# EthanD11/RS-VIO

Hardware: AMD Instinct MI355X
Metric: stereo frames/sec (tracker+BA) on 752×480 EuRoC stream; BA ms/iter at window=10 (higher is better)
Workload: dtype f32 (tracker) / f64 (BA)

## Files before the change

### rs-vio_amd/csrc/ba.hip

```cpp
#include <rccl/rccl.h>

#include <algorithm>
#include <chrono>
#include <cmath>
#include <cstdlib>
#include <cstring>
#include <string>
#include <sys/resource.h>
#include <numeric>
#include <stdexcept>
#include <vector>

#include "common.hpp"

#include "ba_envelope.hpp"
#include "obs_pass.hpp"
#include "se3.hpp"
#include "wave.hpp"

#pragma clang fp contract(fast)

namespace rsvio {

namespace {

RSVIO_DBG_DECL
RSVIO_RT_DECL

constexpr int kMaxFree = 20;
static_assert(kMaxFree == rsvio_env::kMaxFree, "ba_envelope.hpp sizes env[] for the same camera system");
constexpr int kMaxN = 6 * kMaxFree;
enum { RV = 0, RGP = 6, RWR = 9, RUR = 18, RGR = 24, kRawF = 28 };
enum { LV = 0, LG = 6, kLmF = 12 };
// ... 114 lines not shown
    const int* dmap;
};

struct Work {
    double* pose[2];
    double* pw[2];
    const double* pose_init;
    const double* pw_init;
    double* raws[2];
    double* rawl[2];
    int* singular;
    const int* p2p_err;
    double* partA;
    double* partD;
    double* cpart;
    double* sys;
    double* dc;
    double* trial4;
    const LmState* st_prev;
    LmState* st;
    unsigned long long* tick;
};

__device__ __forceinline__ size_t sys_len(const Geometry& G) { return (size_t)G.n_pb * 36 + 12 * G.n_free + 2; }

constexpr int kP2PMax = 8;
constexpr int kP2PMsg = 8192;

struct P2P {
    double* peer[kP2PMax];
    int nranks, rank;
    int* xnw;
    int ll;
};

constexpr int kP2PWaves = 16384;
constexpr size_t kP2PTval = (size_t)2 * kP2PMax * kP2PMsg + 2 * kP2PMax;
constexpr size_t kP2PTflag = kP2PTval + (size_t)2 * kP2PMax * kP2PWaves * 4;
constexpr int kP2PLLMax = 16;
constexpr size_t kP2PLL = kP2PTflag + (size_t)2 * kP2PMax * kP2PWaves;
constexpr size_t kP2PLLSys = kP2PLL + (size_t)2 * kP2PMax * 2 * kP2PLLMax;
constexpr size_t kP2PBytes = sizeof(double) * (kP2PLLSys + (size_t)2 * kP2PMax * 2 * kP2PMsg);

__device__ __forceinline__ unsigned long long* p2p_flags(double* xbuf) {
    return reinterpret_cast<unsigned long long*>(xbuf + (size_t)2 * kP2PMax * kP2PMsg);
}
// ... 183 lines not shown
#pragma unroll
            for (int c = a; c < 3; ++c) L.V[k++] += wt * (J[0][a] * J[0][c] + J[1][a] * J[1][c]);
            L.gp[a] += J[0][a] * wr0 + J[1][a] * wr1;
        }
        if (fr) {
            int u = 0;
#pragma unroll
            for (int a = 0; a < 3; ++a) {
#pragma unroll
                for (int c = 0; c < 3; ++c) L.Wr[a * 3 + c] += wt * (J[0][6 + a] * J[0][c] + J[1][6 + a] * J[1][c]);
#pragma unroll
                for (int c = a; c < 3; ++c) L.Ur[u++] += wt * (J[0][6 + a] * J[0][6 + c] + J[1][6 + a] * J[1][6 + c]);
                L.gr[a] += J[0][6 + a] * wr0 + J[1][6 + a] * wr1;
            }
        }
    }
}

__device__ __forceinline__ void wave_sync() {
    __builtin_amdgcn_fence(__ATOMIC_SEQ_CST, "wavefront");
    __builtin_amdgcn_wave_barrier();
}

template <bool WAVE = false>
__device__ void store_linearization(const Work& Wk, int buf, int s, int lane, bool act, bool fr, int first, int nk,
                                    int l, const SlotLin& L, double (*sh)[64]) {
    if (act && fr) {
        double rec[kRawF];
#pragma unroll
        for (int i = 0; i < 6; ++i) rec[RV + i] = L.V[i];
#pragma unroll
        for (int i = 0; i < 3; ++i) rec[RGP + i] = L.gp[i];
#pragma unroll
        for (int i = 0; i < 9; ++i) rec[RWR + i] = L.Wr[i];
#pragma unroll
        for (int i = 0; i < 6; ++i) rec[RUR + i] = L.Ur[i];
#pragma unroll
        for (int i = 0; i < 3; ++i) rec[RGR + i] = L.gr[i];
        rec[27] = 0.0;
        double2* dst = reinterpret_cast<double2*>(Wk.raws[buf] + (size_t)s * kRawF);
#pragma unroll
        for (int i = 0; i < kRawF / 2; ++i) dst[i] = make_double2(rec[2 * i], rec[2 * i + 1]);
    }
#pragma unroll
    for (int i = 0; i < 6; ++i) sh[i][lane] = L.V[i];
#pragma unroll
    for (int i = 0; i < 3; ++i) sh[6 + i][lane] = L.gp[i];
    if constexpr (WAVE) wave_sync(); else __syncthreads();
// ... 178 lines not shown
        scan(R, true, base);
    }
    for (int i = total + tid; i < G.pair_stride; i += 256) out[i] = make_int4(-1, 0, 0, 0);
}

__global__ __launch_bounds__(256) void ba_stage_in(const uint4* src, uint4* __restrict__ dst, int n_words) {
    const int t = (int)(blockIdx.x * 256 + threadIdx.x), st = (int)(gridDim.x * 256);
    const int i0 = t, i1 = t + st;
    uint4 a, b;
    host_load2x16(src + min(i0, n_words - 1), src + min(i1, n_words - 1), a, b);
    if (i0 < n_words) dst[i0] = a;
    if (i1 < n_words) dst[i1] = b;
}

__global__ __launch_bounds__(256) void ba_build_layout(Geometry G, Prob Pr, SlotSrc S, int nb_slots, int4* hdr,
                                                       double2* huv, int4* pairs) {
    const int b = blockIdx.x;
    if (b < nb_slots)
        build_slots_body(G, Pr, S, hdr, huv, b);
    else
        build_pairs_body(G, Pr, S, pairs, b - nb_slots);
}

__device__ void linearize_body(const Geometry& G, const Prob& Pr, const Work& Wk, int w, int with_reset,
                               double lambda0) {
    __shared__ double sh[10][64];
    const int lane = threadIdx.x;
    const int s = 64 * w + lane;
    if (with_reset) {
        const int nt = G.n_wave * 64;
        for (int i = s; i < 7 * G.n_kf; i += nt) {
            Wk.pose[0][i] = Wk.pose_init[i];
            Wk.pose[1][i] = Wk.pose_init[i];
        }
        for (int i = s; i < 3 * G.n_lm; i += nt) {
            Wk.pw[0][i] = Wk.pw_init[i];
            Wk.pw[1][i] = Wk.pw_init[i];
        }
        if (s == 0) {
            Wk.tick[1] = wall_clock64();
            *Wk.singular = 0;
            LmState st{};
            st.lambda = lambda0;
            st.nu = 2.0;
            *Wk.st = st;
        }
    }
// ... 10 lines not shown
        const Pose P = pose_from7(pose0 + 7 * kf);
        const double* pwp = pw0 + 3 * l;
        const double p[3] = {pwp[0], pwp[1], pwp[2]};
        slot_linearize(G, P, p, h1.y, h1.z, uvq, fr, L);
    } else {
        const Pose P{};
        const double p[3] = {0.0, 0.0, 1.0};
        slot_linearize(G, P, p, 0, 0, uvq, false, L);
    }
    STAMP(12);
    store_linearization(Wk, 0, s, lane, act, fr, first, nk, l, L, sh);
    const double c = wave_sum_det(L.cost);
    if (lane == 0) {
        Wk.partA[w * kPartA] = c;
        Wk.partA[w * kPartA + 1] = 0.0;
    }
    STAMP(14);
}

__global__ __launch_bounds__(64) void ba_linearize(Geometry G, Prob Pr, Work Wk, double lambda0) {
    linearize_body(G, Pr, Wk, blockIdx.x, 1, lambda0);
}

__device__ void trial_scalars_wave(const Geometry& G, const Prob& Pr, const Work& Wk, const LmState& s,
                                   int include_poses, double out[4]) {
    const int lane = threadIdx.x & 63;
    constexpr int kU = 8;
    double4 pv[kU];
    const int wl = max(G.n_wave - 1, 0), el = 7 * G.n_kf - 1;
#pragma unroll
    for (int k = 0; k < kU; ++k)
        pv[k] = *reinterpret_cast<const double4*>(Wk.partD + (size_t)min(lane + 64 * k, wl) * kPartD);
    double p0[3], p1[3];
    int fi[3];
#pragma unroll
    for (int k = 0; k < 3; ++k) {
        const int e = min(lane + 64 * k, el);
        fi[k] = Pr.free_idx[e / 7];
        p0[k] = Wk.pose[0][e];
        p1[k] = Wk.pose[1][e];
    }
#pragma unroll
    for (int k = 0; k < kU; ++k)
        if (lane + 64 * k >= G.n_wave) pv[k] = make_double4(0.0, 0.0, 0.0, 0.0);
    bool fr[3];
#pragma unroll
    for (int k = 0; k < 3; ++k) fr[k] = include_poses && lane + 64 * k <= el && fi[k] >= 0;
// ... 121 lines not shown
                s.nu = 2.0;
                s.cost = s.new_cost;
            } else {
                s.lambda *= s.nu;
                s.nu *= 2.0;
                if (s.lambda > 1e32) {
                    s.status = RSVIO_LM_TRUST_REGION;
                    s.done = 1;
                }
            }
        }
    }
    if (!s.done && s.iter >= max_iter) {
        s.status = RSVIO_LM_MAX_ITERATIONS;
        s.done = 1;
    }
}

struct LmArgs {
    int max_iter;
    double cost_tol, param_tol;
};

__device__ LmState lm_decide(const Geometry& G, const Prob& Pr, const Work& Wk, const LmState* src, int pre_reduced,
                             const LmArgs& la, const P2P* PP = nullptr, const unsigned long long* xgen = nullptr,
                             int* err = nullptr) {
    LmState s = *src;
    double tv[4];
    if (pre_reduced == 4) {
        const int lane = threadIdx.x & 63, r = lane >> 2, i = lane & 3, nr = PP->nranks;
        const unsigned long long gen = *xgen;
        const unsigned g32 = (unsigned)gen;
        const unsigned long long* wv = p2p_ll(PP->peer[PP->rank], (int)(gen & 1), min(r, nr - 1)) + 2 * i;
        unsigned long long a = __hip_atomic_load(wv, __ATOMIC_RELAXED, __HIP_MEMORY_SCOPE_SYSTEM);
        unsigned long long b = __hip_atomic_load(wv + 1, __ATOMIC_RELAXED, __HIP_MEMORY_SCOPE_SYSTEM);
        for (int k = 0; k < 4; ++k) tv[k] = 0.0;
        if (s.pending && !s.done && s.solve_ok) {
            long long spins = 0;
            bool late = false;
            while (r < nr && !((unsigned)(a >> 32) == g32 && (unsigned)(b >> 32) == g32)) {
                if (++spins > (1ll << 25)) {
                    late = true;
                    break;
                }
                __builtin_amdgcn_s_sleep(1);
                a = __hip_atomic_load(wv, __ATOMIC_RELAXED, __HIP_MEMORY_SCOPE_SYSTEM);
                b = __hip_atomic_load(wv + 1, __ATOMIC_RELAXED, __HIP_MEMORY_SCOPE_SYSTEM);
            }
            if (late) atomicExch(err, 1);
            const double got = late ? 0.0 : __longlong_as_double((long long)((a & 0xffffffffull) | (b << 32)));
            for (int k = 0; k < 4; ++k) {
                double v = 0.0;
                for (int q = 0; q < nr; ++q) v += rl64(got, 4 * q + k);
                tv[k] = v;
            }
        }
    } else if (pre_reduced == 2) {
        const unsigned long long gen = *xgen;
        for (int k = 0; k < 4; ++k) tv[k] = 0.0;
        if (s.pending && !s.done && s.solve_ok) trial_scalars_p2p(G, Pr, Wk, s, *PP, gen, err, tv);
    } else if (pre_reduced) {
        for (int k = 0; k < 4; ++k) tv[k] = Wk.trial4[k];
    } else {
        trial_scalars_wave(G, Pr, Wk, s, 1, tv);
    }
    const double cost0 = Wk.sys[(size_t)G.n_pb * 36 + 12 * G.n_free];
    __asm__ volatile("" ::"v"(tv[0]), "v"(tv[1]), "v"(tv[2]), "v"(tv[3]), "v"(cost0));
    STAMP(29);
    if (s.pending && !s.done) {
        const double cost = s.iter == 0 ? cost0 : s.cost;
        lm_update(s, cost, tv, la.max_iter, la.cost_tol, la.param_tol);
        s.pending = 0;
    }
    return s;
}

__device__ __forceinline__ void slot_w(const double* rec, double W[18]) {
    const double* v = rec + RV;
    const double Vs[9] = {v[0], v[1], v[2], v[1], v[3], v[4], v[2], v[4], v[5]};
#pragma unroll
    for (int i = 0; i < 9; ++i) W[i] = Vs[i];
#pragma unroll
    for (int i = 0; i < 9; ++i) W[9 + i] = rec[RWR + i];
}

template <bool DIAG>
__device__ __forceinline__ void schur_pair(const Work& Wk, int cur, double lambda, int chol, int sa, int sb, int l,
                                           double (&acc)[kBlockF]) {
    const double2* ra = reinterpret_cast<const double2*>(Wk.raws[cur] + (size_t)sa * kRawF);
    const double2* rb = reinterpret_cast<const double2*>(Wk.raws[cur] + (size_t)sb * kRawF);
    const double2* rl = reinterpret_cast<const double2*>(Wk.rawl[cur] + (size_t)l * kLmF);
    constexpr int NA = DIAG ? kRawF / 2 : 9;
    double Ra[2 * NA], Rb[18], Lm[10];
#pragma unroll
    for (int i = 0; i < NA; ++i) {
        const double2 x = ra[i];
        Ra[2 * i] = x.x; Ra[2 * i + 1] = x.y;
    }
    if constexpr (!DIAG)
#pragma unroll
        for (int i = 0; i < 9; ++i) {
            const double2 y = rb[i];
            Rb[2 * i] = y.x; Rb[2 * i + 1] = y.y;
        }
#pragma unroll
    for (int i = 0; i < 5; ++i) {
        const double2 x = rl[i];
        Lm[2 * i] = x.x; Lm[2 * i + 1] = x.y;
    }
    double Wa[18], Wb[18];
// ... 25 lines not shown
            for (int c = 0; c < 3; ++c) {
                U[a * 6 + c] = Wa[a * 3 + c];
                U[(3 + a) * 6 + c] = Wa[(3 + a) * 3 + c];
                U[c * 6 + 3 + a] = Wa[(3 + a) * 3 + c];
            }
        const double* ur = Ra + RUR;
        const double Ur[9] = {ur[0], ur[1], ur[2], ur[1], ur[3], ur[4], ur[2], ur[4], ur[5]};
#pragma unroll
        for (int a = 0; a < 3; ++a)
#pragma unroll
            for (int c = 0; c < 3; ++c) U[(3 + a) * 6 + 3 + c] = Ur[a * 3 + c];
#pragma unroll
        for (int i = 0; i < 36; ++i) acc[i] += U[i];
#pragma unroll
        for (int a = 0; a < 6; ++a) {
            const double gca = a < 3 ? Ra[RGP + a] : Ra[RGR + a - 3];
            const double yg = fma(Ya[a * 3 + 2], Lm[LG + 2], fma(Ya[a * 3 + 1], Lm[LG + 1], Ya[a * 3] * Lm[LG]));
            acc[36 + a] += yg - gca;
            acc[42 + a] += gca;
        }
    }
}

template <bool DIAG>
__device__ __forceinline__ void schur_chunk_pairs(const Geometry& G, const Work& Wk, const LmState& s, const int4* pr,
                                                  int4 p1, int tid, double (&acc)[kBlockF]) {
    if (p1.x >= 0) schur_pair<DIAG>(Wk, s.cur, s.lambda, G.chol, p1.x, p1.y, p1.z, acc);
    for (int p = tid + kSchurThreads; p < G.pair_stride; p += kSchurThreads) {
        const int4 q = pr[p];
        if (q.x >= 0) schur_pair<DIAG>(Wk, s.cur, s.lambda, G.chol, q.x, q.y, q.z, acc);
    }
}

__device__ void schur_chunks_body(const Geometry& G, const Prob& Pr, const Work& Wk, const LmArgs& la,
                                  int pre_reduced, int c, const P2P* PP = nullptr,
                                  const unsigned long long* xgen = nullptr, int* err = nullptr) {
    __shared__ double red[kSchurThreads / 64][kBlockF];
    const int tid = threadIdx.x, lane = tid & 63, wave = tid >> 6;
    const int pb = c / kGrp, x = c % kGrp;
    RTSTAMP(0);
    STAMP(26);
    if (G.env_on) {
        int a = 0, r = pb;
        while (a < G.n_free && r >= G.n_free - a) {
            r -= G.n_free - a;
            ++a;
        }
        if (a < G.n_free && a + r > (int)G.env[a]) {
            if (tid < 36) Wk.cpart[(size_t)x * sys_len(G) + pb * 36 + tid] = 0.0;
            return;
        }
    }
    const int4* pr = Pr.pairs + (size_t)c * G.pair_stride;
    const int4 p1 = tid < G.pair_stride ? pr[tid] : make_int4(-1, 0, 0, 0);
    const int fa = Pr.pb_fa[pb];
    const bool diag = fa == Pr.pb_fb[pb];
    __shared__ LmState sd;
// ... 269 lines not shown
            const double piv = rl64(a[0], 0);
            bad = !(piv > 0.0) || !isfinite(piv);
            inv = rcp_f64(piv);
        }
        int seen = 0;
        double uq[CW];
#pragma unroll
        for (int jj = 0; jj < CW; ++jj) uq[jj] = 0.0;
        chol_pipe_step<NP, CW, WV, 0>(a, lane, Lc, Uc, progress, seen, bad, inv, uq, 0.0);
    }
    if (lane == 0) badw[WV] = bad ? 1 : 0;
#ifdef RSVIO_STAMPS
    if (lane == 0) g_dbg[24 + WV] = (unsigned long long)clock64();
#endif
}

__device__ __forceinline__ void k5_result(LmState* st, int ok, double d2, double gd) {
    st->solve_ok = ok;
    st->dc2 = d2;
    st->gcdc = gd;
    st->pending = 1;
}

template <int NF>
__device__ void k5_finish(const Geometry& G, const Work& Wk, double* A, double x, double gcl_v, int n, int lane,
                          const double (&p7)[7], int fidx) {
    LmState* st = Wk.st;
    const double d2 = wave_sum_det(x * x);
    const double gd = wave_sum_det(lane < n ? gcl_v * x : 0.0);
    __builtin_amdgcn_wave_barrier();
    if (lane < n) {
        Wk.dc[lane] = x;
        A[lane] = x;
    }
    __builtin_amdgcn_s_waitcnt(0xc07f);
    __builtin_amdgcn_wave_barrier();
    STAMP(4);
    if (lane < G.n_kf) {
        double* q = Wk.pose[1 - st->cur] + 7 * lane;
        if (fidx < 0) {
#pragma unroll
            for (int i = 0; i < 7; ++i) q[i] = p7[i];
        } else {
            double qv[7];
            se3_plus(p7, A + 6 * fidx, qv);
#pragma unroll
            for (int i = 0; i < 7; ++i) q[i] = qv[i];
        }
// ... 173 lines not shown
    static constexpr int NT = NP / 16 + 1;
    static constexpr int NPP = 16 * NT;
    static constexpr int NH = (NP + kMfPanel - 1) / kMfPanel;
};

constexpr int kMfMapLambda = 1 << 30;
inline void mf_dense_map(int nf, int n_pb, const int* pb_fa, const int* pb_fb, int* map, int np_target = 0,
                         int ld = kMfLd) {
    const int np = np_target > 0 ? np_target : 6 * nf;
    for (int pb = 0; pb < n_pb; ++pb)
        for (int k = 0; k < 36; ++k) {
            const int ra = k / 6, ca = k % 6, fa = pb_fa[pb], fb = pb_fb[pb];
            int v;
            if (fa == fb)
                v = ra >= ca ? ((6 * fa + ca) * ld + 6 * fa + ra) | (ra == ca ? kMfMapLambda : 0) : -1;
            else
                v = (6 * fa + ra) * ld + 6 * fb + ca;
            map[36 * pb + k] = v;
        }
    for (int i = 0; i < 6 * nf; ++i) map[36 * n_pb + i] = i * ld + np;
    for (int i = 0; i < 6 * nf; ++i) map[36 * n_pb + 6 * nf + i] = -2 - i;
}

template <int NF>
__device__ bool combine_mapped(const Geometry& G, const Prob& Pr, const Work& Wk, double* M, double* gsh,
                               const LmState* st, int* fail) {
    constexpr int NE = (NF * (NF + 1) / 2) * 36 + 12 * NF;
    constexpr int T = kK5Threads, kE = (NE + T - 1) / T;
    const size_t L = sys_len(G);
    const int ne = G.n_pb * 36 + 12 * G.n_free;
    const int tid = threadIdx.x;
    double v[kE][kGrp];
    int dst[kE];
#pragma unroll
    for (int i = 0; i < kE; ++i) {
        const int e = tid + T * i, ec = min(e, ne - 1);
        const int d = Pr.dmap[ec];
        dst[i] = e < ne ? d : -1;
#pragma unroll
        for (int x = 0; x < kGrp; ++x) v[i][x] = Wk.cpart[(size_t)x * L + ec];
    }
    double pa[16];
    int sing = 0;
    if (tid < 64) {
        const int wl = max(G.n_wave - 1, 0);
#pragma unroll
        for (int k = 0; k < 16; ++k) pa[k] = Wk.partA[min(tid + 64 * k, wl) * kPartA];
        sing = *Wk.singular;
    }
    const int done = st->done;
    const double lambda = st->lambda;
#pragma unroll
    for (int i = 0; i < kE; ++i)
#pragma unroll
        for (int x = 0; x < kGrp; ++x) __asm__ volatile("" ::"v"(v[i][x]));
    if (done) return true;
#pragma unroll
    for (int i = 0; i < kE; ++i) {
        double a = v[i][0];
#pragma unroll
        for (int x = 1; x < kGrp; ++x) a += v[i][x];
        const int d = dst[i];
        if (d >= 0) {
            if (d & kMfMapLambda) a += lambda;
            M[d & (kMfMapLambda - 1)] = a;
        } else if (d <= -2) {
            gsh[-2 - d] = a;
        }
    }
    if (tid < 64) {
        double c = 0.0;
#pragma unroll
        for (int k = 0; k < 16; ++k) c += tid + 64 * k < G.n_wave ? pa[k] : 0.0;
        for (int w = tid + 64 * 16; w < G.n_wave; w += 64) c += Wk.partA[w * kPartA];
        c = wave_sum_det(c);
        if (tid == 0) {
            Wk.sys[G.n_pb * 36 + 12 * G.n_free] = c;
            *fail = sing;
        }
    }
    return false;
}

template <int NF>
__device__ bool combine_p2p_ll(const Geometry& G, const Work& Wk, double* M, double* gsh, int* fail, const P2P& P,
                               unsigned long long* xgen, int* err,
                               const double (&v)[((NF * (NF + 1) / 2) * 36 + 12 * NF + kK5Threads - 1) / kK5Threads][kGrp],
                               const int (&dst)[((NF * (NF + 1) / 2) * 36 + 12 * NF + kK5Threads - 1) / kK5Threads],
                               const double (&pa)[16], int sing, double lambda, unsigned long long gen) {
    constexpr int NE = (NF * (NF + 1) / 2) * 36 + 12 * NF;
    constexpr int T = kK5Threads, kE = (NE + T - 1) / T;
    const int ne = G.n_pb * 36 + 12 * G.n_free;
// ... 514 lines not shown
    } else {
        bk_update<NF, K, NW - 1>(M, U + (K & 1) * 6 * LD, lane, wave - 1, env[K]);
    }
    if constexpr (K + 1 < NF) bk_steps<NF, K + 1, NW, KD>(M, U, Dsc, Lsc, a, tid, bad, env, Dv);
}

template <int NF, int NW, bool KD = false>
__device__ __forceinline__ void bk_factor(double* M, double* U, double* S, int tid, bool& bad,
                                          const unsigned char* env, double* Dv = nullptr) {
    using D = BkDims<NF>;
    double a[D::RPL][6];
    if ((tid >> 6) == 0) {
        const int lane = tid & 63;
#pragma unroll
        for (int h = 0; h < D::RPL; ++h) {
            const int r = lane + 64 * h < D::NPP ? lane + 64 * h : D::NPP - 1;
#pragma unroll
            for (int j = 0; j < 6; ++j) a[h][j] = M[j * D::LD + r];
        }
    }
    bk_steps<NF, 0, NW, KD>(M, U, S, S + 36, a, tid, bad, env, Dv);
}

template <int NF, bool LL = false>
__device__ void camera_solve_mfma_body(const Geometry& G, const Prob& Pr, const Work& Wk, int combine,
                                       const P2P* P = nullptr, unsigned long long* xgen = nullptr, int* err = nullptr) {
    static_assert(NF >= 1 && NF <= 10, "one row per lane: n <= 60");
    constexpr int NP = MfDims<NF>::NP, NPP = MfDims<NF>::NPP;
    __shared__ __attribute__((aligned(16))) double M[NPP * kMfLd];
    __shared__ __attribute__((aligned(16))) double Lf[NPP * kMfLd];
    __shared__ __attribute__((aligned(16))) double Up[2 * kMfPanel * kMfLd];
    __shared__ double gsh[NP];
    __shared__ int fail;
    RTSTAMP(4);
    LmState* st = Wk.st;
    const int tid = threadIdx.x, lane = tid & 63, wave = tid >> 6;
    const int nF = G.n_free, n = 6 * nF;
    const int SC0 = G.n_pb * 36 + 12 * nF;
    double p7b[2][7];
    int fidx = -1;
    if (wave == 0 && lane < G.n_kf) {
        fidx = Pr.free_idx[lane];
#pragma unroll
        for (int b = 0; b < 2; ++b)
#pragma unroll
            for (int i = 0; i < 7; ++i) p7b[b][i] = Wk.pose[b][7 * lane + i];
    } else {
#pragma unroll
        for (int b = 0; b < 2; ++b)
#pragma unroll
            for (int i = 0; i < 7; ++i) p7b[b][i] = i == 3 ? 1.0 : 0.0;
    }
    STAMP(0);
    if (combine == 2) {
        if (combine_p2p<NF, LL>(G, Pr, Wk, M, gsh, st, &fail, *P, xgen, err)) return;
    } else if (combine) {
        if (combine_mapped<NF>(G, Pr, Wk, M, gsh, st, &fail)) return;
    } else {
        if (st->done) return;
        const double* sys = Wk.sys;
        const int ne = G.n_pb * 36 + 12 * nF;
        for (int e = tid; e < ne; e += kK5Threads) {
            const int d = Pr.dmap[e];
            if (d >= 0)
                M[d & (kMfMapLambda - 1)] = sys[e];
            else if (d <= -2)
                gsh[-2 - d] = sys[e];
        }
        if (tid == 0) fail = sys[SC0 + 1] != 0.0;
    }
    const int cur = st->cur;
    double p7[7];
#pragma unroll
    for (int i = 0; i < 7; ++i) p7[i] = cur ? p7b[1][i] : p7b[0][i];
    if (n < NP) {
        for (int e = tid; e < NP * (NP + 1); e += kK5Threads) {
            const int c = e / (NP + 1), r = e - c * (NP + 1);
            if (r >= c && ((r >= n && r < NP) || (c >= n && c < NP))) M[c * kMfLd + r] = r == c ? 1.0 : 0.0;
// ... 33 lines not shown
        const double m = Lres[lj * kMfLd + j];
        lt[j] = lane < j ? m : 0.0;
    }
#pragma unroll
    for (int j = NP - 1; j >= 0; --j) yv = fma(-lt[j], rl64(yv, j), yv);
    STAMP(3);
    k5_finish<NF>(G, Wk, Up, lane < n ? yv : 0.0, gcl_v, n, lane, p7, fidx);
    RTSTAMP(5);
}

template <int NF>
__global__ __launch_bounds__(kK5Threads) void ba_camera_solve_mfma(Geometry G, Prob Pr, Work Wk, int combine) {
    camera_solve_mfma_body<NF>(G, Pr, Wk, combine);
}

template <int NF, bool LL>
__global__ __launch_bounds__(kK5Threads) void ba_camera_solve_mfma_p2p(Geometry G, Prob Pr, Work Wk, P2P P,
                                                                        unsigned long long* xgen, int* err) {
    camera_solve_mfma_body<NF, LL>(G, Pr, Wk, 2, &P, xgen, err);
}

constexpr int kBkWaves = 8;

template <int NF>
__device__ __forceinline__ void camera_solve_blk_body(const Geometry& G, const Prob& Pr, const Work& Wk, int combine) {
    using D = BkDims<NF>;
    constexpr int NP = D::NP, LD = D::LD;
    static_assert(NF > 10 && D::RPL == 2 && D::NPP <= LD, "the 11..20 free-keyframe solver");
    constexpr int T = 64 * kBkWaves;
    __shared__ __attribute__((aligned(16))) double M[16 * D::NTC * LD];
    __shared__ __attribute__((aligned(16))) double U[2 * 6 * LD];
    __shared__ __attribute__((aligned(16))) double S[72];
    __shared__ double gsh[NP];
    __shared__ double dcs[128];
    __shared__ int fail;
    LmState* st = Wk.st;
    const int tid = threadIdx.x, lane = tid & 63, wave = tid >> 6;
    const int nF = G.n_free, n = 6 * nF;
    const int ne = G.n_pb * 36 + 12 * nF;
    STAMP(0);
    double p7b[2][7];
    int fidx = -1;
#pragma unroll
    for (int b = 0; b < 2; ++b)
#pragma unroll
        for (int i = 0; i < 7; ++i) p7b[b][i] = i == 3 ? 1.0 : 0.0;
    if (wave == 0 && lane < G.n_kf) {
        fidx = Pr.free_idx[lane];
// ... 443 lines not shown
#pragma unroll
            for (int i = 0; i < 7; ++i) qd[i] = p7[i];
        } else {
            double qv[7];
            se3_plus(p7, dcs + 6 * fidx, qv);
#pragma unroll
            for (int i = 0; i < 7; ++i) qd[i] = qv[i];
        }
    }
    if (lane == 0) k5_result(st, 1, d2, gd);
    STAMP(5);
}

#ifndef RSVIO_EXPORT_FENCE
#define RSVIO_EXPORT_FENCE 0
#endif
__device__ __forceinline__ void export_done() {
#if RSVIO_EXPORT_FENCE
    __builtin_amdgcn_fence(__ATOMIC_RELEASE, "");
#else
    __builtin_amdgcn_s_waitcnt(kWaitStores);
#endif
}
template <bool FUSED, bool LAST = false>
__device__ void k6_body(const Geometry& G, const Prob& Pr, const Work& Wk, int w, int lane, double (*sh)[64],
                        double (*shp)[64], double (*shs)[64], const P2P* PP = nullptr,
                        unsigned long long gen = 0, unsigned long long* k6tag = nullptr,
                        unsigned long long* k6part = nullptr, double* hout = nullptr) {
    const int s = 64 * w + lane;
    const int4 h0 = Pr.slot_hdr[2 * s], h1 = Pr.slot_hdr[2 * s + 1];
    const double2 uvq[2] = {Pr.slot_uv[2 * s], Pr.slot_uv[2 * s + 1]};
    const LmState* st = Wk.st;
    const bool act = h1.y > 0;
    const int kf = h0.x, l = h0.y, first = act ? h0.z : lane, nk = act ? h0.w : 1;
    const bool fr = h1.x >= 0;
    const int kfc = act ? kf : 0, lc = act ? l : 0, fc = (act && fr) ? h1.x : 0;
    double recb[2][18], Lmb[2][10], pcb[2][3], p7b[2][7], d6[6];
#pragma unroll
    for (int b = 0; b < 2; ++b) {
        const double2* wr = reinterpret_cast<const double2*>(Wk.raws[b] + (size_t)s * kRawF);
#pragma unroll
        for (int i = 0; i < 9; ++i) {
            const double2 x = wr[i];
            recb[b][2 * i] = x.x; recb[b][2 * i + 1] = x.y;
        }
        const double2* lr = reinterpret_cast<const double2*>(Wk.rawl[b] + (size_t)lc * kLmF);
#pragma unroll
        for (int i = 0; i < 5; ++i) {
// ... 408 lines not shown
        if (threadIdx.x == 0) __hip_atomic_store(k6cnt, 0u, __ATOMIC_RELAXED, __HIP_MEMORY_SCOPE_AGENT);
        k6_last_push(G, Pr, Wk, P, xgen, gen, k6part, s);
    } else {
        const LmState s = *Wk.st;
        if (s.done || !s.solve_ok) return;
        k6_last_push(G, Pr, Wk, P, xgen, gen, k6part, s);
    }
}

__global__ __launch_bounds__(64) void ba_reduce_trial(Geometry G, Prob Pr, Work Wk, int include_poses) {
    const LmState s = *Wk.st;
    if (s.done) return;
    double v[4];
    trial_scalars_wave(G, Pr, Wk, s, include_poses, v);
    if (threadIdx.x == 0)
        for (int k = 0; k < 4; ++k) Wk.trial4[k] = v[k];
}

constexpr int kK7Threads = 256;
#ifndef RSVIO_K7_BLOCKS
#define RSVIO_K7_BLOCKS 16
#endif
constexpr int kK7Blocks = RSVIO_K7_BLOCKS;
__device__ __forceinline__ void lm_decide_body(const Geometry& G, const Prob& Pr, const Work& Wk, int pre_reduced,
                                               const LmArgs& la, LmState* host, unsigned long long* htick,
                                               double* hout, const P2P* PP = nullptr,
                                               const unsigned long long* xgen = nullptr, int* err = nullptr) {
    STAMP(8);
    __shared__ LmState sd;
    unsigned long long xstamp = 0, xcur = 0, stamp = 0;
    if (hout) {
        stamp = Wk.tick[1];
        xstamp = Wk.tick[2];
        xcur = Wk.tick[3];
        __asm__ volatile("" ::"v"(stamp), "v"(xstamp), "v"(xcur));
    }
    if (threadIdx.x < 64) {
        const LmState d = lm_decide(G, Pr, Wk, Wk.st_prev, pre_reduced, la, PP, xgen, err);
        if (threadIdx.x == 0) {
            sd = d;
            if (blockIdx.x == 0) {
                LmState h = d;
                h.p2p_err = Wk.p2p_err ? *Wk.p2p_err : 0;
                *Wk.st = d;
                *host = h;
            }
        }
// ... 27 lines not shown
        const unsigned long long t = Wk.tick[0] + 1;
        Wk.tick[0] = t;
        htick[1] = Wk.tick[1];
        htick[2] = wall_clock64();
        __threadfence_system();
        __hip_atomic_store(htick, t, __ATOMIC_RELEASE, __HIP_MEMORY_SCOPE_SYSTEM);
    }
    STAMP(10);
}

__global__ __launch_bounds__(kK7Threads) void ba_lm_decide(Geometry G, Prob Pr, Work Wk, int pre_reduced, LmArgs la,
                                                           LmState* host, unsigned long long* htick, double* hout) {
    lm_decide_body(G, Pr, Wk, pre_reduced, la, host, htick, hout);
}

__global__ __launch_bounds__(kK7Threads) void ba_lm_decide_p2p(Geometry G, Prob Pr, Work Wk, LmArgs la, LmState* host,
                                                               unsigned long long* htick, double* hout, P2P P,
                                                               const unsigned long long* xgen, int* err, int mode) {
    lm_decide_body(G, Pr, Wk, mode, la, host, htick, hout, &P, xgen, err);
}

struct WinDesc {
    Geometry G;
    Prob Pr;
    Work W[4];
    int skip;
};

__device__ __forceinline__ void desc_touch1(const void* p) { __asm__ volatile("" ::"s"(p)); }
template <class... T>
__device__ __forceinline__ void desc_touch(const T*... p) {
    (desc_touch1(p), ...);
}


__global__ __launch_bounds__(64) void bab_linearize(const WinDesc* __restrict__ D, double lambda0) {
    const WinDesc& d = D[blockIdx.y];
    const int skip = d.skip, bound = d.G.n_wave;
    const Prob Pr = d.Pr;
    const Work& Wk = d.W[2];
    desc_touch(Pr.slot_hdr, Pr.slot_uv, Wk.pose_init, Wk.pw_init, Wk.st);
    if (skip | ((int)blockIdx.x >= bound)) return;
    linearize_body(d.G, Pr, Wk, blockIdx.x, 1, lambda0);
}

__global__ __launch_bounds__(kSchurThreads) void bab_schur_chunks(const WinDesc* __restrict__ D, int wi, LmArgs la) {
    const WinDesc& d = D[blockIdx.y];
    const int skip = d.skip, bound = d.G.n_chunk;
    const Prob Pr = d.Pr;
    const Work& Wk = d.W[wi];
    desc_touch(Pr.pairs, Wk.partD, Wk.pose[0], Wk.pose[1], Wk.st_prev, Wk.st);
    if (skip | ((int)blockIdx.x >= bound)) return;
    schur_chunks_body(d.G, Pr, Wk, la, 0, blockIdx.x);
}

template <int NF>
__global__ __launch_bounds__(kK5Threads) void bab_camera_solve(const WinDesc* __restrict__ D, int wi) {
    const WinDesc& d = D[blockIdx.x];
    const int skip = d.skip, nkf = d.G.n_kf, nf = d.G.n_free, npb = d.G.n_pb, nw = d.G.n_wave;
    const Prob Pr = d.Pr;
    const Work& Wk = d.W[wi];
    desc_touch(Pr.free_idx, Pr.dmap, Wk.pose[0], Wk.pose[1], Wk.cpart, Wk.partA, Wk.singular, Wk.st);
    __asm__ volatile("" ::"s"(nkf), "s"(nf), "s"(npb), "s"(nw));
    if (skip) return;
    camera_solve_mfma_body<NF>(d.G, Pr, Wk, 1);
}

template <int NF>
__global__ __launch_bounds__(64 * kBkWaves) void bab_camera_solve_blk(const WinDesc* __restrict__ D, int wi) {
    const WinDesc& d = D[blockIdx.x];
    const int skip = d.skip;
    const Prob Pr = d.Pr;
    const Work& Wk = d.W[wi];
    desc_touch(Pr.free_idx, Pr.dmap, Wk.pose[0], Wk.pose[1], Wk.cpart, Wk.partA, Wk.singular, Wk.st);
    if (skip) return;
    camera_solve_blk_body<NF>(d.G, Pr, Wk, 1);
}

__global__ __launch_bounds__(64) void bab_backsub_relinearize(const WinDesc* __restrict__ D, int wi) {
    const WinDesc& d = D[blockIdx.y];
    const int skip = d.skip, bound = d.G.n_wave;
    const Prob Pr = d.Pr;
    const Work& Wk = d.W[wi];
    desc_touch(Pr.slot_hdr, Pr.slot_uv, Wk.st, Wk.raws[0], Wk.raws[1], Wk.rawl[0], Wk.rawl[1], Wk.pw[0], Wk.pw[1],
               Wk.pose[0], Wk.pose[1], Wk.dc);
    if (skip | ((int)blockIdx.x >= bound)) return;
    __shared__ double sh[10][64];
    __shared__ double shp[3][64];
    __shared__ double shs[4][64];
    k6_body<false>(d.G, Pr, Wk, blockIdx.x, threadIdx.x, sh, shp, shs);
}

__global__ __launch_bounds__(64) void bab_backsub_trial_export(const WinDesc* __restrict__ D, int wi, double* hout) {
    const WinDesc& d = D[blockIdx.y];
    const int skip = d.skip, bound = d.G.n_wave;
    const Prob Pr = d.Pr;
    const Work& Wk = d.W[wi];
    desc_touch(Pr.slot_hdr, Pr.slot_uv, Wk.st, Wk.raws[0], Wk.raws[1], Wk.rawl[0], Wk.rawl[1], Wk.pw[0], Wk.pw[1],
               Wk.pose[0], Wk.pose[1], Wk.dc, Wk.tick);
    if (skip | ((int)blockIdx.x >= bound)) return;
    __shared__ double sh[10][64];
    __shared__ double shp[3][64];
    __shared__ double shs[4][64];
    k6_body<false, true>(d.G, Pr, Wk, blockIdx.x, threadIdx.x, sh, shp, shs, nullptr, 0, nullptr, nullptr, hout);
}

__global__ __launch_bounds__(kK7Threads) void bad_lm_decide(const WinDesc* __restrict__ D, int wi, LmArgs la,
                                                            LmState* host, unsigned long long* htick, double* hout) {
    const WinDesc& d = D[0];
    const Prob Pr = d.Pr;
    const Work& Wk = d.W[wi];
    lm_decide_body(d.G, Pr, Wk, 0, la, host, htick, hout);
}

__global__ __launch_bounds__(64) void bab_lm_decide(const WinDesc* __restrict__ D, int wi, LmArgs la, LmState* host) {
    const WinDesc& d = D[blockIdx.x];
    if (d.skip) return;
    const LmState s = lm_decide(d.G, d.Pr, d.W[wi], d.W[wi].st, 0, la);
    if (threadIdx.x == 0) {
        *d.W[wi].st = s;
        host[blockIdx.x] = s;
    }
}


__device__ void p2p_exchange(const double* msg, int n, const P2P& P, unsigned long long* xgen, int* err, double* out,
                             unsigned long long gen_pre = 0) {
    __shared__ unsigned long long sgen;
    const int tid = threadIdx.x, nr = P.nranks, me = P.rank;
    if (!gen_pre) {
        if (tid == 0) sgen = *xgen + 1;
        __syncthreads();
    }
    const unsigned long long gen = gen_pre ? gen_pre : sgen;
// ... 179 lines not shown
    WinDesc hdesc{};
    double desc_huber = std::nan("");
    int desc_chol = -1;
    HostBuf<WinDesc> h_desc1;
    hipEvent_t ev_desc = nullptr;
    bool desc_pending = false;
    bool desc_mode() const { return desc_on && coll == 0 && k5_variant == 2 && G.n_free <= 10 && G.n_wave > 0; }
    int fold_lvl = 3;
    int fold_req = 3;
    bool p2p_shared_gpu = false;
    bool p2p_fold() const { return fold_lvl >= 1 && coll == 2 && k5_variant == 2 && G.n_free <= 10; }
    bool p2p_fold2() const { return fold_lvl == 2 && p2p_fold(); }
    bool p2p_fold3() const { return fold_lvl == 3 && p2p_fold() && k6_fits(); }
    int k6_cap = 0;
    bool k6_fits() const { return G.n_wave + 1 <= k6_cap; }
    int p2p_share = 1;
    bool p2p_fold4() const { return fold_lvl == 4 && p2p_fold(); }
    const WinDesc* dptr() const { return reinterpret_cast<const WinDesc*>(d_arena.p + lay.desc); }
    void fill_desc(WinDesc& d) const {
        d = WinDesc{};
        d.G = G;
        d.G.huber_delta = desc_huber;
        d.G.chol = desc_chol;
        d.Pr = prob();
        d.W[0] = work(0);
        d.W[1] = work(1);
        d.W[2] = work_at(0);
        d.W[3] = work_at(1);
        d.skip = 0;
    }
    void refresh_desc() {
        if (desc_pending && hipEventQuery(ev_desc) != hipSuccess) {
            (void)hipGetLastError();
            RSVIO_HIP(hipEventSynchronize(ev_desc));
        }
        desc_pending = false;
        desc_huber = G.huber_delta;
        desc_chol = G.chol;
        hdesc.G.huber_delta = desc_huber;
        hdesc.G.chol = desc_chol;
        if (!h_desc1.p) h_desc1.alloc(1);
        *h_desc1.p = hdesc;
        settled = false;
        RSVIO_HIP(hipMemcpyAsync(d_arena.p + lay.desc, h_desc1.p, sizeof(WinDesc), hipMemcpyHostToDevice, stream));
        RSVIO_HIP(hipEventRecord(ev_desc, stream));
        desc_pending = true;
    }
    bool start_graph(const rsvio_lm_cfg& cfg, int& k) {
        if (coll == 1 || !graphs_ok) return false;
        const bool dm = desc_mode() && solves_of_problem == 0;
        ++solves_of_problem;
// ... 1427 lines not shown
            const Geometry& G = w.G;
            skip[i] = (G.n_obs < 6 || G.n_obs < G.n_kf + G.n_lm || G.n_wave == 0) ? 1 : 0;
            if (skip[i]) continue;
            ++active;
            nf = std::max(nf, G.n_free);
            max_wave = std::max(max_wave, G.n_wave);
            max_chunk = std::max(max_chunk, G.n_chunk);
            ne_total += (size_t)36 * G.n_pb + 12 * G.n_free;
        }
        if (nf > 10) nf = bk_template_nf(nf);
        max_wave = (max_wave + kGrp - 1) / kGrp * kGrp;
        if (h_dmap.n < std::max<size_t>(ne_total, 1)) {
            h_dmap.alloc(ne_total + 1);
            d_dmap.alloc(ne_total + 1);
        }
        size_t off = 0;
        for (int i = 0; i < B; ++i) {
            BundleAdjuster& w = *win[i];
            WinDesc& d = h_desc.p[i];
            d.skip = skip[i];
            d.G = w.G;
            d.G.huber_delta = cfg.huber_delta;
            d.G.chol = cfg.linear_solver == RSVIO_SOLVER_CHOLESKY ? 1 : 0;
            d.Pr = w.prob();
            d.W[0] = w.work(0);
            d.W[1] = w.work(1);
            d.W[2] = w.work_at(0);
            d.W[3] = w.work_at(1);
            if (skip[i]) continue;
            const size_t ne = (size_t)36 * w.G.n_pb + 12 * w.G.n_free;
            mf_dense_map(w.G.n_free, w.G.n_pb, w.hs_pb_fa.data(), w.hs_pb_fb.data(), h_dmap.p + off, 6 * nf,
                         nf > 10 ? kBkLd : kMfLd);
            d.Pr.dmap = d_dmap.p + off;
            off += ne;
        }
        for (int i = 0; i < B; ++i) {
            if (skip[i]) {
                res[i] = rsvio_ba_result{};
                res[i].status = RSVIO_LM_SKIPPED;
            }
        }
        if (!active) return;
        for (int i = 0; i < B; ++i) {
            BundleAdjuster& w = *win[i];
            if (w.settled) continue;
            RSVIO_HIP(hipEventRecord(ev_win[i], w.stream));
            RSVIO_HIP(hipStreamWaitEvent(stream, ev_win[i], 0));
        }
        RSVIO_HIP(hipMemcpyAsync(d_dmap.p, h_dmap.p, sizeof(int) * std::max<size_t>(off, 1), hipMemcpyHostToDevice, stream));
        RSVIO_HIP(hipMemcpyAsync(d_desc.p, h_desc.p, sizeof(WinDesc) * B, hipMemcpyHostToDevice, stream));
        RSVIO_HIP(hipEventRecord(ev0, stream));
        hipLaunchKernelGGL(bab_linearize, dim3(max_wave, B), dim3(64), 0, stream, d_desc.p, cfg.lambda_init);
        RSVIO_HIP(hipGetLastError());
        const LmArgs la{cfg.max_iterations, cfg.cost_tolerance, cfg.parameter_tolerance};
        const int max_it = std::max(cfg.max_iterations, 1);
        int enq = 0;
// ... 335 lines not shown
```

Baseline: 5108.

## Type descriptor pointers as global address space and pair-load combine entries

Wraps the batched descriptor's Prob/Work pointers in a gptr view that casts to address_space(1), so device code emits global loads instead of flat loads. The kernels become templated on the pointer view. combine_mapped now loads two entries per thread as int2/double2 when the entry count allows, which halves the number of load instructions. The NF==2 camera solve also gets a waves_per_eu hint. The risks are higher register pressure from the widened per-thread arrays, and the p2p paths are compiled out for the global-view types.

After: 5218, median of 6. 2.1% higher.

```diff
diff --git a/rs-vio_amd/csrc/ba.hip b/rs-vio_amd/csrc/ba.hip
--- a/rs-vio_amd/csrc/ba.hip
+++ b/rs-vio_amd/csrc/ba.hip
@@ -3,12 +3,14 @@
 #include <algorithm>
 #include <chrono>
 #include <cmath>
+#include <cstddef>
 #include <cstdlib>
 #include <cstring>
 #include <string>
 #include <sys/resource.h>
 #include <numeric>
 #include <stdexcept>
+#include <type_traits>
 #include <vector>
 
 #include "common.hpp"
@@ -169,6 +171,68 @@
     unsigned long long* tick;
 };
 
+template <class T>
+struct gptr {
+    T* p;
+    __device__ __forceinline__ T* get() const {
+#if defined(__HIP_DEVICE_COMPILE__) && !defined(RSVIO_DESC_FLAT)
+        return (T*)(T __attribute__((address_space(1)))*)(unsigned long long)p;
+#else
+        return p;
+#endif
+    }
+    __device__ __forceinline__ operator T*() const { return get(); }
+    __device__ __forceinline__ T* operator->() const { return get(); }
+};
+
+struct ProbG {
+    gptr<const int> free_idx;
+    gptr<const int4> slot_hdr;
+    gptr<const double2> slot_uv;
+    gptr<const int4> pairs;
+    gptr<const int> pb_fa;
+    gptr<const int> pb_fb;
+    gptr<const int> dmap;
+};
+
+struct WorkG {
+    gptr<double> pose[2];
+    gptr<double> pw[2];
+    gptr<const double> pose_init;
+    gptr<const double> pw_init;
+    gptr<double> raws[2];
+    gptr<double> rawl[2];
+    gptr<int> singular;
+    gptr<const int> p2p_err;
+    gptr<double> partA;
+    gptr<double> partD;
+    gptr<double> cpart;
+    gptr<double> sys;
+    gptr<double> dc;
+    gptr<double> trial4;
+    gptr<const LmState> st_prev;
+    gptr<LmState> st;
+    gptr<unsigned long long> tick;
+};
+
+static_assert(sizeof(ProbG) == sizeof(Prob) && alignof(ProbG) == alignof(Prob) && sizeof(WorkG) == sizeof(Work) &&
+                  alignof(WorkG) == alignof(Work) && std::is_trivially_copyable<ProbG>::value &&
+                  std::is_trivially_copyable<WorkG>::value,
+              "the descriptor's views are Prob / Work with typed pointers");
+static_assert(offsetof(ProbG, dmap) == offsetof(Prob, dmap) && offsetof(WorkG, raws) == offsetof(Work, raws) &&
+                  offsetof(WorkG, singular) == offsetof(Work, singular) && offsetof(WorkG, st) == offsetof(Work, st) &&
+                  offsetof(WorkG, tick) == offsetof(Work, tick),
+              "field for field");
+inline ProbG global_view(const Prob& p) {
+    ProbG g;
+    std::memcpy(&g, &p, sizeof g);
+    return g;
+}
+inline WorkG global_view(const Work& w) {
+    WorkG g;
+    std::memcpy(&g, &w, sizeof g);
+    return g;
+}
 __device__ __forceinline__ size_t sys_len(const Geometry& G) { return (size_t)G.n_pb * 36 + 12 * G.n_free + 2; }
 
 constexpr int kP2PMax = 8;
@@ -398,8 +462,8 @@
     __builtin_amdgcn_wave_barrier();
 }
 
-template <bool WAVE = false>
-__device__ void store_linearization(const Work& Wk, int buf, int s, int lane, bool act, bool fr, int first, int nk,
+template <bool WAVE = false, class WkT>
+__device__ void store_linearization(const WkT& Wk, int buf, int s, int lane, bool act, bool fr, int first, int nk,
                                     int l, const SlotLin& L, double (*sh)[64]) {
     if (act && fr) {
         double rec[kRawF];
@@ -624,7 +688,8 @@
         build_pairs_body(G, Pr, S, pairs, b - nb_slots);
 }
 
-__device__ void linearize_body(const Geometry& G, const Prob& Pr, const Work& Wk, int w, int with_reset,
+template <class PrT, class WkT>
+__device__ void linearize_body(const Geometry& G, const PrT& Pr, const WkT& Wk, int w, int with_reset,
                                double lambda0) {
     __shared__ double sh[10][64];
     const int lane = threadIdx.x;
@@ -681,7 +746,8 @@
     linearize_body(G, Pr, Wk, blockIdx.x, 1, lambda0);
 }
 
-__device__ void trial_scalars_wave(const Geometry& G, const Prob& Pr, const Work& Wk, const LmState& s,
+template <class PrT, class WkT>
+__device__ void trial_scalars_wave(const Geometry& G, const PrT& Pr, const WkT& Wk, const LmState& s,
                                    int include_poses, double out[4]) {
     const int lane = threadIdx.x & 63;
     constexpr int kU = 8;
@@ -849,7 +915,8 @@
     double cost_tol, param_tol;
 };
 
-__device__ LmState lm_decide(const Geometry& G, const Prob& Pr, const Work& Wk, const LmState* src, int pre_reduced,
+template <class PrT, class WkT>
+__device__ LmState lm_decide(const Geometry& G, const PrT& Pr, const WkT& Wk, const LmState* src, int pre_reduced,
                              const LmArgs& la, const P2P* PP = nullptr, const unsigned long long* xgen = nullptr,
                              int* err = nullptr) {
     LmState s = *src;
@@ -885,7 +952,8 @@
     } else if (pre_reduced == 2) {
         const unsigned long long gen = *xgen;
         for (int k = 0; k < 4; ++k) tv[k] = 0.0;
-        if (s.pending && !s.done && s.solve_ok) trial_scalars_p2p(G, Pr, Wk, s, *PP, gen, err, tv);
+        if constexpr (std::is_same<WkT, Work>::value)
+            if (s.pending && !s.done && s.solve_ok) trial_scalars_p2p(G, Pr, Wk, s, *PP, gen, err, tv);
     } else if (pre_reduced) {
         for (int k = 0; k < 4; ++k) tv[k] = Wk.trial4[k];
     } else {
@@ -911,8 +979,8 @@
     for (int i = 0; i < 9; ++i) W[9 + i] = rec[RWR + i];
 }
 
-template <bool DIAG>
-__device__ __forceinline__ void schur_pair(const Work& Wk, int cur, double lambda, int chol, int sa, int sb, int l,
+template <bool DIAG, class WkT>
+__device__ __forceinline__ void schur_pair(const WkT& Wk, int cur, double lambda, int chol, int sa, int sb, int l,
                                            double (&acc)[kBlockF]) {
     const double2* ra = reinterpret_cast<const double2*>(Wk.raws[cur] + (size_t)sa * kRawF);
     const double2* rb = reinterpret_cast<const double2*>(Wk.raws[cur] + (size_t)sb * kRawF);
@@ -984,8 +1052,8 @@
     }
 }
 
-template <bool DIAG>
-__device__ __forceinline__ void schur_chunk_pairs(const Geometry& G, const Work& Wk, const LmState& s, const int4* pr,
+template <bool DIAG, class WkT>
+__device__ __forceinline__ void schur_chunk_pairs(const Geometry& G, const WkT& Wk, const LmState& s, const int4* pr,
                                                   int4 p1, int tid, double (&acc)[kBlockF]) {
     if (p1.x >= 0) schur_pair<DIAG>(Wk, s.cur, s.lambda, G.chol, p1.x, p1.y, p1.z, acc);
     for (int p = tid + kSchurThreads; p < G.pair_stride; p += kSchurThreads) {
@@ -994,7 +1062,8 @@
     }
 }
 
-__device__ void schur_chunks_body(const Geometry& G, const Prob& Pr, const Work& Wk, const LmArgs& la,
+template <class PrT, class WkT>
+__device__ void schur_chunks_body(const Geometry& G, const PrT& Pr, const WkT& Wk, const LmArgs& la,
                                   int pre_reduced, int c, const P2P* PP = nullptr,
                                   const unsigned long long* xgen = nullptr, int* err = nullptr) {
     __shared__ double red[kSchurThreads / 64][kBlockF];
@@ -1310,8 +1379,8 @@
     st->pending = 1;
 }
 
-template <int NF>
-__device__ void k5_finish(const Geometry& G, const Work& Wk, double* A, double x, double gcl_v, int n, int lane,
+template <int NF, class WkT>
+__device__ void k5_finish(const Geometry& G, const WkT& Wk, double* A, double x, double gcl_v, int n, int lane,
                           const double (&p7)[7], int fidx) {
     LmState* st = Wk.st;
     const double d2 = wave_sum_det(x * x);
@@ -1531,23 +1600,51 @@
     for (int i = 0; i < 6 * nf; ++i) map[36 * n_pb + 6 * nf + i] = -2 - i;
 }
 
-template <int NF>
-__device__ bool combine_mapped(const Geometry& G, const Prob& Pr, const Work& Wk, double* M, double* gsh,
+#ifdef RSVIO_K5_PULL8
+constexpr bool kK5Pairs = false;
+#else
+constexpr bool kK5Pairs = true;
+#endif
+template <int NF, class PrT, class WkT>
+__device__ bool combine_mapped(const Geometry& G, const PrT& Pr, const WkT& Wk, double* M, double* gsh,
                                const LmState* st, int* fail) {
     constexpr int NE = (NF * (NF + 1) / 2) * 36 + 12 * NF;
-    constexpr int T = kK5Threads, kE = (NE + T - 1) / T;
+    constexpr int T = kK5Threads;
+    constexpr int W = kK5Pairs && NE > T ? 2 : 1;
+    static_assert(NE % W == 0, "entry pairs");
+    constexpr int kE = (NE / W + T - 1) / T;
     const size_t L = sys_len(G);
     const int ne = G.n_pb * 36 + 12 * G.n_free;
     const int tid = threadIdx.x;
-    double v[kE][kGrp];
-    int dst[kE];
+    int done = 0;
+    double lambda = 0.0;
+    if constexpr (W == 2) {
+        done = st->done;
+        lambda = st->lambda;
+    }
+    double v[kE][kGrp][W];
+    int dst[kE][W];
 #pragma unroll
     for (int i = 0; i < kE; ++i) {
-        const int e = tid + T * i, ec = min(e, ne - 1);
-        const int d = Pr.dmap[ec];
-        dst[i] = e < ne ? d : -1;
-#pragma unroll
-        for (int x = 0; x < kGrp; ++x) v[i][x] = Wk.cpart[(size_t)x * L + ec];
+        if constexpr (W == 2) {
+            const int np = ne >> 1, q = tid + T * i, qc = min(q, np - 1);
+            const int2 d = reinterpret_cast<const int2*>(static_cast<const int*>(Pr.dmap))[qc];
+            dst[i][0] = q < np ? d.x : -1;
+            dst[i][1] = q < np ? d.y : -1;
+            const double2* const row = reinterpret_cast<const double2*>(static_cast<const double*>(Wk.cpart)) + qc;
+#pragma unroll
+            for (int x = 0; x < kGrp; ++x) {
+                const double2 t = row[(size_t)x * (L >> 1)];
+                v[i][x][0] = t.x;
+                v[i][x][1] = t.y;
+            }
+        } else {
+            const int e = tid + T * i, ec = min(e, ne - 1);
+            const int d = Pr.dmap[ec];
+            dst[i][0] = e < ne ? d : -1;
+#pragma unroll
+            for (int x = 0; x < kGrp; ++x) v[i][x][0] = Wk.cpart[(size_t)x * L + ec];
+        }
     }
     double pa[16];
     int sing = 0;
@@ -1557,26 +1654,32 @@
         for (int k = 0; k < 16; ++k) pa[k] = Wk.partA[min(tid + 64 * k, wl) * kPartA];
         sing = *Wk.singular;
     }
-    const int done = st->done;
-    const double lambda = st->lambda;
+    if constexpr (W == 1) {
+        done = st->done;
+        lambda = st->lambda;
+    }
 #pragma unroll
     for (int i = 0; i < kE; ++i)
 #pragma unroll
-        for (int x = 0; x < kGrp; ++x) __asm__ volatile("" ::"v"(v[i][x]));
+        for (int x = 0; x < kGrp; ++x)
+#pragma unroll
+            for (int k = 0; k < W; ++k) __asm__ volatile("" ::"v"(v[i][x][k]));
     if (done) return true;
 #pragma unroll
-    for (int i = 0; i < kE; ++i) {
-        double a = v[i][0];
-#pragma unroll
-        for (int x = 1; x < kGrp; ++x) a += v[i][x];
-        const int d = dst[i];
-        if (d >= 0) {
-            if (d & kMfMapLambda) a += lambda;
-            M[d & (kMfMapLambda - 1)] = a;
-        } else if (d <= -2) {
-            gsh[-2 - d] = a;
-        }
-    }
+    for (int i = 0; i < kE; ++i)
+#pragma unroll
+        for (int k = 0; k < W; ++k) {
+            double a = v[i][0][k];
+#pragma unroll
+            for (int x = 1; x < kGrp; ++x) a += v[i][x][k];
+            const int d = dst[i][k];
+            if (d >= 0) {
+                if (d & kMfMapLambda) a += lambda;
+                M[d & (kMfMapLambda - 1)] = a;
+            } else if (d <= -2) {
+                gsh[-2 - d] = a;
+            }
+        }
     if (tid < 64) {
         double c = 0.0;
 #pragma unroll
@@ -2137,8 +2240,8 @@
     bk_steps<NF, 0, NW, KD>(M, U, S, S + 36, a, tid, bad, env, Dv);
 }
 
-template <int NF, bool LL = false>
-__device__ void camera_solve_mfma_body(const Geometry& G, const Prob& Pr, const Work& Wk, int combine,
+template <int NF, bool LL = false, class PrT, class WkT>
+__device__ void camera_solve_mfma_body(const Geometry& G, const PrT& Pr, const WkT& Wk, int combine,
                                        const P2P* P = nullptr, unsigned long long* xgen = nullptr, int* err = nullptr) {
     static_assert(NF >= 1 && NF <= 10, "one row per lane: n <= 60");
     constexpr int NP = MfDims<NF>::NP, NPP = MfDims<NF>::NPP;
@@ -2168,7 +2271,9 @@
     }
     STAMP(0);
     if (combine == 2) {
-        if (combine_p2p<NF, LL>(G, Pr, Wk, M, gsh, st, &fail, *P, xgen, err)) return;
+        if constexpr (std::is_same<WkT, Work>::value) {
+            if (combine_p2p<NF, LL>(G, Pr, Wk, M, gsh, st, &fail, *P, xgen, err)) return;
+        }
     } else if (combine) {
         if (combine_mapped<NF>(G, Pr, Wk, M, gsh, st, &fail)) return;
     } else {
@@ -2248,8 +2353,8 @@
 
 constexpr int kBkWaves = 8;
 
-template <int NF>
-__device__ __forceinline__ void camera_solve_blk_body(const Geometry& G, const Prob& Pr, const Work& Wk, int combine) {
+template <int NF, class PrT, class WkT>
+__device__ __forceinline__ void camera_solve_blk_body(const Geometry& G, const PrT& Pr, const WkT& Wk, int combine) {
     using D = BkDims<NF>;
     constexpr int NP = D::NP, LD = D::LD;
     static_assert(NF > 10 && D::RPL == 2 && D::NPP <= LD, "the 11..20 free-keyframe solver");
@@ -2739,8 +2844,8 @@
     __builtin_amdgcn_s_waitcnt(kWaitStores);
 #endif
 }
-template <bool FUSED, bool LAST = false>
-__device__ void k6_body(const Geometry& G, const Prob& Pr, const Work& Wk, int w, int lane, double (*sh)[64],
+template <bool FUSED, bool LAST = false, class PrT, class WkT>
+__device__ void k6_body(const Geometry& G, const PrT& Pr, const WkT& Wk, int w, int lane, double (*sh)[64],
                         double (*shp)[64], double (*shs)[64], const P2P* PP = nullptr,
                         unsigned long long gen = 0, unsigned long long* k6tag = nullptr,
                         unsigned long long* k6part = nullptr, double* hout = nullptr) {
@@ -3195,7 +3300,8 @@
 #define RSVIO_K7_BLOCKS 16
 #endif
 constexpr int kK7Blocks = RSVIO_K7_BLOCKS;
-__device__ __forceinline__ void lm_decide_body(const Geometry& G, const Prob& Pr, const Work& Wk, int pre_reduced,
+template <class PrT, class WkT>
+__device__ __forceinline__ void lm_decide_body(const Geometry& G, const PrT& Pr, const WkT& Wk, int pre_reduced,
                                                const LmArgs& la, LmState* host, unsigned long long* htick,
                                                double* hout, const P2P* PP = nullptr,
                                                const unsigned long long* xgen = nullptr, int* err = nullptr) {
@@ -3269,23 +3375,23 @@
 
 struct WinDesc {
     Geometry G;
-    Prob Pr;
-    Work W[4];
+    ProbG Pr;
+    WorkG W[4];
     int skip;
 };
 
 __device__ __forceinline__ void desc_touch1(const void* p) { __asm__ volatile("" ::"s"(p)); }
 template <class... T>
-__device__ __forceinline__ void desc_touch(const T*... p) {
-    (desc_touch1(p), ...);
+__device__ __forceinline__ void desc_touch(gptr<T>... p) {
+    (desc_touch1(p.p), ...);
 }
 
 
 __global__ __launch_bounds__(64) void bab_linearize(const WinDesc* __restrict__ D, double lambda0) {
     const WinDesc& d = D[blockIdx.y];
     const int skip = d.skip, bound = d.G.n_wave;
-    const Prob Pr = d.Pr;
-    const Work& Wk = d.W[2];
+    const ProbG Pr = d.Pr;
+    const WorkG& Wk = d.W[2];
     desc_touch(Pr.slot_hdr, Pr.slot_uv, Wk.pose_init, Wk.pw_init, Wk.st);
     if (skip | ((int)blockIdx.x >= bound)) return;
     linearize_body(d.G, Pr, Wk, blockIdx.x, 1, lambda0);
@@ -3294,19 +3400,20 @@
 __global__ __launch_bounds__(kSchurThreads) void bab_schur_chunks(const WinDesc* __restrict__ D, int wi, LmArgs la) {
     const WinDesc& d = D[blockIdx.y];
     const int skip = d.skip, bound = d.G.n_chunk;
-    const Prob Pr = d.Pr;
-    const Work& Wk = d.W[wi];
+    const ProbG Pr = d.Pr;
+    const WorkG& Wk = d.W[wi];
     desc_touch(Pr.pairs, Wk.partD, Wk.pose[0], Wk.pose[1], Wk.st_prev, Wk.st);
     if (skip | ((int)blockIdx.x >= bound)) return;
     schur_chunks_body(d.G, Pr, Wk, la, 0, blockIdx.x);
 }
 
 template <int NF>
-__global__ __launch_bounds__(kK5Threads) void bab_camera_solve(const WinDesc* __restrict__ D, int wi) {
+__global__ __launch_bounds__(kK5Threads) __attribute__((amdgpu_waves_per_eu(NF == 2 ? 5 : 1)))
+void bab_camera_solve(const WinDesc* __restrict__ D, int wi) {
     const WinDesc& d = D[blockIdx.x];
     const int skip = d.skip, nkf = d.G.n_kf, nf = d.G.n_free, npb = d.G.n_pb, nw = d.G.n_wave;
-    const Prob Pr = d.Pr;
-    const Work& Wk = d.W[wi];
+    const ProbG Pr = d.Pr;
+    const WorkG& Wk = d.W[wi];
     desc_touch(Pr.free_idx, Pr.dmap, Wk.pose[0], Wk.pose[1], Wk.cpart, Wk.partA, Wk.singular, Wk.st);
     __asm__ volatile("" ::"s"(nkf), "s"(nf), "s"(npb), "s"(nw));
     if (skip) return;
@@ -3317,8 +3424,8 @@
 __global__ __launch_bounds__(64 * kBkWaves) void bab_camera_solve_blk(const WinDesc* __restrict__ D, int wi) {
     const WinDesc& d = D[blockIdx.x];
     const int skip = d.skip;
-    const Prob Pr = d.Pr;
-    const Work& Wk = d.W[wi];
+    const ProbG Pr = d.Pr;
+    const WorkG& Wk = d.W[wi];
     desc_touch(Pr.free_idx, Pr.dmap, Wk.pose[0], Wk.pose[1], Wk.cpart, Wk.partA, Wk.singular, Wk.st);
     if (skip) return;
     camera_solve_blk_body<NF>(d.G, Pr, Wk, 1);
@@ -3327,8 +3434,8 @@
 __global__ __launch_bounds__(64) void bab_backsub_relinearize(const WinDesc* __restrict__ D, int wi) {
     const WinDesc& d = D[blockIdx.y];
     const int skip = d.skip, bound = d.G.n_wave;
-    const Prob Pr = d.Pr;
-    const Work& Wk = d.W[wi];
+    const ProbG Pr = d.Pr;
+    const WorkG& Wk = d.W[wi];
     desc_touch(Pr.slot_hdr, Pr.slot_uv, Wk.st, Wk.raws[0], Wk.raws[1], Wk.rawl[0], Wk.rawl[1], Wk.pw[0], Wk.pw[1],
                Wk.pose[0], Wk.pose[1], Wk.dc);
     if (skip | ((int)blockIdx.x >= bound)) return;
@@ -3341,8 +3448,8 @@
 __global__ __launch_bounds__(64) void bab_backsub_trial_export(const WinDesc* __restrict__ D, int wi, double* hout) {
     const WinDesc& d = D[blockIdx.y];
     const int skip = d.skip, bound = d.G.n_wave;
-    const Prob Pr = d.Pr;
-    const Work& Wk = d.W[wi];
+    const ProbG Pr = d.Pr;
+    const WorkG& Wk = d.W[wi];
     desc_touch(Pr.slot_hdr, Pr.slot_uv, Wk.st, Wk.raws[0], Wk.raws[1], Wk.rawl[0], Wk.rawl[1], Wk.pw[0], Wk.pw[1],
                Wk.pose[0], Wk.pose[1], Wk.dc, Wk.tick);
     if (skip | ((int)blockIdx.x >= bound)) return;
@@ -3355,8 +3462,8 @@
 __global__ __launch_bounds__(kK7Threads) void bad_lm_decide(const WinDesc* __restrict__ D, int wi, LmArgs la,
                                                             LmState* host, unsigned long long* htick, double* hout) {
     const WinDesc& d = D[0];
-    const Prob Pr = d.Pr;
-    const Work& Wk = d.W[wi];
+    const ProbG Pr = d.Pr;
+    const WorkG& Wk = d.W[wi];
     lm_decide_body(d.G, Pr, Wk, 0, la, host, htick, hout);
 }
 
@@ -3582,11 +3689,11 @@
         d.G = G;
         d.G.huber_delta = desc_huber;
         d.G.chol = desc_chol;
-        d.Pr = prob();
-        d.W[0] = work(0);
-        d.W[1] = work(1);
-        d.W[2] = work_at(0);
-        d.W[3] = work_at(1);
+        d.Pr = global_view(prob());
+        d.W[0] = global_view(work(0));
+        d.W[1] = global_view(work(1));
+        d.W[2] = global_view(work_at(0));
+        d.W[3] = global_view(work_at(1));
         d.skip = 0;
     }
     void refresh_desc() {
@@ -5060,16 +5167,16 @@
             d.G = w.G;
             d.G.huber_delta = cfg.huber_delta;
             d.G.chol = cfg.linear_solver == RSVIO_SOLVER_CHOLESKY ? 1 : 0;
-            d.Pr = w.prob();
-            d.W[0] = w.work(0);
-            d.W[1] = w.work(1);
-            d.W[2] = w.work_at(0);
-            d.W[3] = w.work_at(1);
+            d.Pr = global_view(w.prob());
+            d.W[0] = global_view(w.work(0));
+            d.W[1] = global_view(w.work(1));
+            d.W[2] = global_view(w.work_at(0));
+            d.W[3] = global_view(w.work_at(1));
             if (skip[i]) continue;
             const size_t ne = (size_t)36 * w.G.n_pb + 12 * w.G.n_free;
             mf_dense_map(w.G.n_free, w.G.n_pb, w.hs_pb_fa.data(), w.hs_pb_fb.data(), h_dmap.p + off, 6 * nf,
                          nf > 10 ? kBkLd : kMfLd);
-            d.Pr.dmap = d_dmap.p + off;
+            d.Pr.dmap.p = d_dmap.p + off;
             off += ne;
         }
         for (int i = 0; i < B; ++i) {
```
